# citiususc/veryfasttree

Measured on AMD Instinct MI355X. Metric: profile-ops/sec, higher is better.
Workload: dtype f32; 1 GPU; c4_1M_x200_nt_tophits; n_seqs=1000000, n_pos=200, active_nodes=750000, top_k=2000

## Files before the change

veryfasttree_amd/csrc/vft_api.hip:

```cpp
#include <hip/hip_runtime.h>
#include <csignal>
#include <unistd.h>

#include <cmath>
#include <cstdarg>
#include <cstdio>
#include <cstdlib>
#include <cstring>
#include <new>
#include <algorithm>
#include <utility>
#include <vector>
#include <chrono>

#include "../../include/vft_hip.h"
#include "vft_owned.h"
#include "vft_staging.h"
#define VFT_PAIR_STAGE_CAP 2048
#include "vft_kernels_ml.h"

VFT_ML_HEAVY_INSTANCES(extern)
#include "vft_kernels_ml_long.h"
VFT_ML_LONG_INSTANCES(extern)
#include "vft_kernels_nj.h"
// ... 2015 lines not shown
                return fail(c, VFT_ERR_TIMEOUT, "no selection result after %.0f s (the stream is still busy)", c->waitLimitS);
        }
    }
}

template <typename REAL, typename HIT>
static int run_select(vft_ctx *c, int K, const int64_t *queries, int64_t lo, int64_t hi, int32_t k) {
    std::vector<SelSlot> hs((size_t) K);
    for (int s = 0; s < K; s++) {
        const vft_ctx::SweepSlotHost &h = c->slots[(size_t) s];
        SelSlot &d = hs[(size_t) s];
        d.crit = h.swCrit;
        d.dist = h.swDist;
        d.weight = h.swWeight;
        d.partMin = h.partMin;
        d.partMax = h.partMax;
        d.sel = h.sel;
        d.slices = h.slices;
        d.candKey = h.candKey;
        d.candId = h.candId;
        d.hits = h.dRes + sizeof(SelectHeader);
        d.hdr = (SelectHeader *) h.dRes;
        d.hostHdr = (SelectHeader *) h.hResDev;
        d.hostHits = h.hResDev + sizeof(SelectHeader);
        d.query = queries[s];
        d.nPart = h.nPart;
        d.pad = 0;
    }
    Stage st;
    if (int r = st.open(c, hs.size() * sizeof(SelSlot), Stage::RING_ONLY)) return r;
    st.put(0, hs.data(), hs.size() * sizeof(SelSlot));
    const SelSlot *slots = st.dev<const SelSlot>(0);
    auto round = [&](const SelSlot *sl, unsigned ny, int first, int s0) -> int {
        const unsigned long long seq = ++c->signalSeq;
        launch((k_select_hist<REAL>), dim3(VFT_SEL_WGS, ny), dim3(VFT_WG), 0, c->stream, sl, lo, hi, first);
        launch((k_select_collect<REAL>), dim3(VFT_SEL_WGS, ny), dim3(VFT_WG), 0, c->stream, sl, lo, hi, (unsigned int) k);
        launch((k_select_rank<REAL, HIT>), dim3(VFT_CAND_CAP * VFT_RANK_LANES / VFT_WG, ny), dim3(VFT_WG), 0, c->stream, sl, k, lo, hi, (long long) seq);
        LAUNCHCHK(c);
        return wait_headers(c, s0, (int) ny, seq);
    };
    if (int r = round(slots, (unsigned) K, 1, 0)) return r;
    for (int s = 0; s < K; s++) {
        const SelectHeader *h = (const SelectHeader *) c->slots[(size_t) s].hRes;
        for (int level = 0; h->overflow; level++) {
            if (level == VFT_MAX_LEVEL)
                return fail(c, VFT_ERR_STATE, "top-k select: more than %d hits tied at the k-th criterion", VFT_CAND_CAP);
            launch(k_select_refine, dim3(1, 1), dim3(1), 0, c->stream, slots + s);
            if (int r = round(slots + s, 1u, 0, s)) return r;
        }
    }
    return VFT_OK;
}

#ifdef VFT_SELECT_PHASES
extern "C" int vft_debug_select_phases(vft_ctx *c, unsigned long long *out, int64_t nOut) {
    if (nOut != (int64_t) VFT_SELPH_ROWS * VFT_SELPH_SEEDS * VFT_SELPH_MARKS) return fail(c, VFT_ERR_INVALID, "vft_debug_select_phases: %d x %d x %d words", VFT_SELPH_ROWS, VFT_SELPH_SEEDS, VFT_SELPH_MARKS);
    HIPCHK(c, hipStreamSynchronize(c->stream));
    HIPCHK(c, hipMemcpyFromSymbol(out, HIP_SYMBOL(vft_selph), sizeof(vft_selph)));
    static const unsigned long long zero[VFT_SELPH_ROWS][VFT_SELPH_SEEDS][VFT_SELPH_MARKS] = {};
    HIPCHK(c, hipMemcpyToSymbol(HIP_SYMBOL(vft_selph), zero, sizeof(zero)));
    return VFT_OK;
}
#endif

static int sweep_one(vft_ctx *c, int slot, int64_t query, int64_t nActive, int64_t nDiffAllow, double totdiam, bool staged = false) {
    if (int r = flush_pending(c)) return r;
    const int64_t lo = c->shardLo, hi = c->shardHi < c->maxnode ? c->shardHi : c->maxnode;
    if (c->maxStamp - nActive > nDiffAllow)
        if (int r = launch_out_distances(c, nullptr, 0, nActive, nDiffAllow, totdiam, false)) return r;
    if ((int64_t) c->hNOut[query] - nActive > nDiffAllow) {
        if (nActive > c->maxStamp) c->maxStamp = nActive;
        SweepArgs s{};
        s.nActive = nActive;
        s.nDiffAllow = nDiffAllow;
        s.totdiam = totdiam;
        s.force = 0;
        VFT_DISPATCH(c, launch((k_out_distance_one<REAL, NC>), dim3(1), dim3(VFT_WG), pw_lds_bytes(c) / c->pwWaves, c->stream,
                               arena<REAL>(c), query, s));
        LAUNCHCHK(c);
    }
    SweepArgs s{};
    s.query = query;
    s.lo = lo;
    s.hi = hi;
    s.nActive = nActive;
    s.nDiffAllow = nDiffAllow;
    s.totdiam = totdiam;
    s.queryIsLeaf = query < c->d.nSeqs ? 1 : 0;
#ifdef VFT_ABLATE
    if (const char *dbg = getenv("VFT_SWEEP_ABLATE")) s.pad = atoi(dbg);
#endif
    const int64_t span = hi > lo ? hi - lo : 0;
    const bool ntPath = c->cfg.n_codes == 4 && !c->hasDm;
    const unsigned grid = ntPath ? sweep_nt_grid(c, s, !s.queryIsLeaf) : cdiv(span > 0 ? span : 1, VFT_WG);
    c->slots[(size_t) slot].nPart = (int) grid;
    const int64_t nPosPad = (int64_t) c->d.nChunk * VFT_CHUNK;
    if (c->cfg.n_codes == 4 && !c->hasDm) {
        if (c->cfg.precision == 4) {
            const QueryBuf<float> Q = staged ? qbuf_slot<float>(c, slot) : qbuf<float>(c, 0);
            if (!staged) launch((k_extract_query<float, 4>), dim3(cdiv(nPosPad, 256)), dim3(256), 0, c->stream, arena<float>(c), query, Q);
            if (s.queryIsLeaf) launch_sweep_nt<float, MODE_CRIT_LEAFQ>(c, s, grid, Q, true, slot);
            else launch_sweep_nt<float, MODE_CRIT>(c, s, grid, Q, true, slot);
        } else {
            const QueryBuf<double> Q = staged ? qbuf_slot<double>(c, slot) : qbuf<double>(c, 0);
            if (!staged) launch((k_extract_query<double, 4>), dim3(cdiv(nPosPad, 256)), dim3(256), 0, c->stream, arena<double>(c), query, Q);
            if (s.queryIsLeaf) launch_sweep_nt<double, MODE_CRIT_LEAFQ>(c, s, grid, Q, true, slot);
// ... 8 lines not shown
            const unsigned wgrid = (unsigned) std::min<int64_t>(cdiv(span > 0 ? span : 1, c->pwWaves), 256 * 16);
            c->slots[(size_t) slot].nPart = (int) wgrid;
            VFT_DISPATCH(c, (launch((k_sweep_wave<REAL, NC>), dim3(wgrid), dim3(64 * c->pwWaves), pw_lds_bytes(c), c->stream,
                                    arena<REAL>(c), s, sweepout<REAL>(c, slot))));
        } else {
            VFT_DISPATCH(c, (launch((k_sweep_generic<REAL, NC>), dim3(grid), dim3(VFT_WG), 0, c->stream,
                                    arena<REAL>(c), s, sweepout<REAL>(c, slot))));
        }
        kernel_event(c);
        kernel_event(c);
    }
    LAUNCHCHK(c);
    return VFT_OK;
}

template <typename REAL, int S>
static int sweep_group(vft_ctx *c, bool leafSeeds, const int *slotOf, const int64_t *queries, int64_t nActive, int64_t nDiffAllow, double totdiam, const void *mq, const void *lq) {
    SweepArgs s{};
    s.query = queries[slotOf[0]];
    s.lo = c->shardLo;
    s.hi = c->shardHi < c->maxnode ? c->shardHi : c->maxnode;
    s.nActive = nActive;
    s.nDiffAllow = nDiffAllow;
    s.totdiam = totdiam;
    s.queryIsLeaf = leafSeeds ? 1 : 0;
    const unsigned grid = sweep_nt_grid(c, s, !leafSeeds);
    MultiLeafQ<REAL, S> M;
    for (int q = 0; q < S; q++) {
        M.Q[q] = qbuf_slot<REAL>(c, slotOf[q]);
        M.O[q] = sweepout<REAL>(c, slotOf[q]);
        M.query[q] = queries[slotOf[q]];
        c->slots[(size_t) slotOf[q]].nPart = (int) grid;
    }
    M.mq = (const REAL *) mq;
    M.lq = (const uint32_t *) lq;
    kernel_event(c);
    if (grid && leafSeeds) launch((k_sweep_nt_leafq_multi<REAL, S>), dim3(grid), dim3(VFT_WG), 0, c->stream, arena<REAL>(c), M, s);
    if (grid && !leafSeeds) launch((k_sweep_nt_profq_multi<REAL, S>), dim3(grid), dim3(VFT_WG), 0, c->stream, arena<REAL>(c), M, s);
    kernel_event(c);
    kernel_event(c);
    if (c->timeKernels) c->kevSweeps += S - 1;
    LAUNCHCHK(c);
    return VFT_OK;
}

static bool mixed_sweep_fits(vft_ctx *c) {
    SweepArgs s{};
    s.lo = c->shardLo;
    s.hi = c->shardHi < c->maxnode ? c->shardHi : c->maxnode;
    const unsigned grid = sweep_nt_grid(c, s, true);
    if (!s.nLeafWG || grid == (unsigned) s.nLeafWG || s.hi <= s.leafEnd) return false;
    if (c->rs != 4) return false;
    const int64_t N = slot_nodes(c, 1);
    return (int64_t) cdiv(s.leafEnd - s.lo, VFT_WG) + (int64_t) (grid - (unsigned) s.nLeafWG) <= (int64_t) cdiv(N, VFT_WG);
}

template <typename REAL>
static int sweep_mixed(vft_ctx *c, const int *leafPos, const int *profPos, const int64_t *queries, int64_t nActive, int64_t nDiffAllow, double totdiam, const void *mq, const void *lq) {
    constexpr int S = 4;
    MixedArgs<REAL, S, S> a;
    memset((void *) &a, 0, sizeof(a));
    a.A = arena<REAL>(c);
    SweepArgs &s = a.s;
    s.query = queries[profPos[0]];
    s.lo = c->shardLo;
    s.hi = c->shardHi < c->maxnode ? c->shardHi : c->maxnode;
    s.nActive = nActive;
    s.nDiffAllow = nDiffAllow;
    s.totdiam = totdiam;
    s.queryIsLeaf = 0;
    const unsigned gridP = sweep_nt_grid(c, s, true);
    a.nInt = (int32_t) (gridP - (unsigned) s.nLeafWG);
    a.nLeafHeavy = (int32_t) cdiv(s.leafEnd - s.lo, VFT_WG);
    for (int q = 0; q < S; q++) {
        a.M.L.Q[q] = qbuf_slot<REAL>(c, leafPos[q]);
        a.M.L.O[q] = sweepout<REAL>(c, leafPos[q]);
        a.M.L.query[q] = queries[leafPos[q]];
        c->slots[(size_t) leafPos[q]].nPart = a.nLeafHeavy + a.nInt;
        a.M.P.Q[q] = qbuf_slot<REAL>(c, profPos[q]);
        a.M.P.O[q] = sweepout<REAL>(c, profPos[q]);
        a.M.P.query[q] = queries[profPos[q]];
        c->slots[(size_t) profPos[q]].nPart = (int) gridP;
    }
    a.M.L.mq = nullptr;
    a.M.L.lq = (const uint32_t *) lq;
    a.M.P.mq = (const REAL *) mq;
    a.M.P.lq = nullptr;
    kernel_event(c);
    launch((k_sweep_nt_mixed_multi<REAL, S, S>), dim3((unsigned) (a.nInt + a.nLeafHeavy + s.nLeafWG)), dim3(VFT_WG), 0, c->stream, a);
    kernel_event(c);
    kernel_event(c);
    if (c->timeKernels) c->kevSweeps += 2 * S - 1;
    LAUNCHCHK(c);
    return VFT_OK;
}

static int no_slot(vft_ctx *c) { return fail(c, VFT_ERR_STATE, "the context has no sweep buffers (vft_create failed)"); }

static int sweep_args_ok(vft_ctx *c, int64_t query, int64_t nActive, int32_t k) {
    if (c->slots.empty()) return no_slot(c);
    if (!c->leavesUp) return fail(c, VFT_ERR_STATE, "vft_sweep before vft_upload_leaves");
    if (query < 0 || query >= c->maxnode || nActive < 3 || k < 0 || k > c->hitsCap)
        return fail(c, VFT_ERR_INVALID, "vft_sweep: bad arguments (query %lld, nActive %lld, k %d)", (long long) query,
                    (long long) nActive, (int) k);
    return VFT_OK;
}

extern "C" int vft_sweep(vft_ctx *c, int64_t query, int64_t nActive, int64_t nDiffAllow, double totdiam, int32_t k,
                         void *hits, void *dHitsOut, int64_t *bestJ) {
    if (!c) return VFT_ERR_INVALID;
    if (int r = sweep_args_ok(c, query, nActive, k)) return r;
    if (int r = sweep_one(c, 0, query, nActive, nDiffAllow, totdiam)) return r;
    if (k == 0) return VFT_OK;
    if (bestJ && k < 2) return fail(c, VFT_ERR_INVALID, "vft_sweep: best_j needs k >= 2");
    const int64_t lo = c->shardLo, hi = c->shardHi < c->maxnode ? c->shardHi : c->maxnode;
    int r;
    if (c->cfg.precision == 4) r = run_select<float, vft_hit_f32>(c, 1, &query, lo, hi, k);
    else r = run_select<double, vft_hit_f64>(c, 1, &query, lo, hi, k);
    if (r) return r;
    const size_t hb = (size_t) k * (c->cfg.precision == 4 ? sizeof(vft_hit_f32) : sizeof(vft_hit_f64));
    const vft_ctx::SweepSlotHost &h = c->slots[0];
    if (dHitsOut) HIPCHK(c, hipMemcpyAsync(dHitsOut, h.dRes + sizeof(SelectHeader), hb, hipMemcpyDeviceToDevice, c->stream));
    if (hits) memcpy(hits, h.hRes + sizeof(SelectHeader), hb);
    if (bestJ) *bestJ = (int64_t) ((const SelectHeader *) h.hRes)->bestJ;
    return VFT_OK;
}

struct SeedGroup {
    int pos[4];
    int n;
    bool leaf;
};

extern "C" int vft_sweep_batch(vft_ctx *c, int32_t nSeeds, const int64_t *queries, int64_t nActive, int64_t nDiffAllow,
                               double totdiam, int32_t k, void *hits, void *dHitsOut, int64_t *bestJ) {
    if (!c || !queries || nSeeds < 1 || nSeeds > VFT_MAX_SLOTS || k < 1) return VFT_ERR_INVALID;
    if (bestJ && k < 2) return fail(c, VFT_ERR_INVALID, "vft_sweep_batch: best_j needs k >= 2");
    for (int s = 0; s < nSeeds; s++)
        if (int r = sweep_args_ok(c, queries[s], nActive, k)) return r;
    if (int r = ensure_slots(c, nSeeds)) return r;
    const bool staged = c->cfg.n_codes == 4 && !c->hasDm && nSeeds > 1;
    std::vector<SeedGroup> groups;
// ... 2006 lines not shown
```

veryfasttree_amd/csrc/vft_kernels_nj.h:

```cpp
#pragma once
#include "vft_device.h"

#define VFT_WG 256

template <typename REAL>
struct QueryBuf {
    REAL *w;
    uint8_t *code;
    REAL *f;
    uint4 *enc;
    double2 *tab;
};

template <typename REAL>
__device__ __forceinline__ void vft_query_tab(const QueryBuf<REAL> &q, int64_t p, REAL wq, const REAL *f) {
#pragma unroll
    for (int c = 0; c < 5; c++) {
        double2 v = make_double2(0.0, 0.0);
        if (c < 4 && wq > 0) {
            const double wgt = (double) wq;
            const double piece = 1.0 - (double) f[c < 4 ? c : 0];
            v = make_double2(wgt * piece, wgt);
        }
        q.tab[p * 5 + c] = v;
// ... 113 lines not shown
    int64_t query;
    int64_t lo, hi;
    int64_t nActive, nDiffAllow;
    double totdiam;
    int32_t queryIsLeaf;
    int32_t force;
    int32_t nLeafWG;
    int32_t pad;
    int64_t leafEnd;
    int64_t heavyLo;
};

template <typename REAL>
struct SweepOut {
    REAL *dist, *weight, *crit;
    REAL *partMin, *partMax;
};

template <typename REAL, int NWAVES>
__device__ __forceinline__ void vft_block_minmax_n(REAL cmin, REAL cmax, REAL *partMin, REAL *partMax, int part) {
    __shared__ REAL smin[NWAVES], smax[NWAVES];
#pragma unroll
    for (int off = 32; off > 0; off >>= 1) {
        const REAL a = __shfl_xor(cmin, off, 64), b = __shfl_xor(cmax, off, 64);
        cmin = a < cmin ? a : cmin;
        cmax = b > cmax ? b : cmax;
    }
    if ((threadIdx.x & 63) == 0) {
        smin[threadIdx.x >> 6] = cmin;
        smax[threadIdx.x >> 6] = cmax;
    }
    __syncthreads();
    if (threadIdx.x == 0) {
#pragma unroll
        for (int w = 1; w < NWAVES; w++) {
            cmin = smin[w] < cmin ? smin[w] : cmin;
            cmax = smax[w] > cmax ? smax[w] : cmax;
        }
        partMin[part] = cmin;
        partMax[part] = cmax;
    }
}
template <typename REAL>
__device__ __forceinline__ void vft_block_minmax(REAL cmin, REAL cmax, REAL *partMin, REAL *partMax, int part) {
    vft_block_minmax_n<REAL, VFT_WG / 64>(cmin, cmax, partMin, partMax, part);
}

enum { MODE_CRIT = 0, MODE_OUTDIST = 1, MODE_CRIT_LEAFQ = 2 };

__device__ __forceinline__ void vft_seq_counts(const uint4 a, const uint4 b, int &nUse, int &nSame) {
    const uint32_t x = a.x & b.x, y = a.y & b.y, z = a.z & b.z, w = a.w & b.w;
    nUse += __popc(x & 0x10101010u) + __popc(y & 0x10101010u) + __popc(z & 0x10101010u) + __popc(w & 0x10101010u);
    nSame += __popc(x & 0x0F0F0F0Fu) + __popc(y & 0x0F0F0F0Fu) + __popc(z & 0x0F0F0F0Fu) + __popc(w & 0x0F0F0F0Fu);
}

#ifndef VFT_SUB
#define VFT_SUB 8
#endif
__device__ __forceinline__ uint32_t vft_query_code(const uint8_t *code, int64_t p0, int b) {
    const uint32_t w = vft_uniform_load<uint32_t>((const uint32_t *) (code + p0 + (b & ~3)));
    return (w >> ((b & 3) * 8)) & 0xFFu;
}
template <typename REAL>
__device__ __forceinline__ uint32_t vft_query_code(const QueryBuf<REAL> &Q, int64_t p0, int b) {
    return vft_query_code(Q.code, p0, b);
}

template <typename REAL, bool QLEAF>
struct IntChunk {
    REAL w[VFT_SUB];
    REAL f[VFT_SUB][QLEAF ? 1 : 4];
};

typedef unsigned int __attribute__((ext_vector_type(4))) vft_u4_t;
typedef unsigned int __attribute__((ext_vector_type(2))) vft_u2_t;
typedef const __attribute__((address_space(4))) vft_u4_t *vft_smask_t;
typedef const __attribute__((address_space(4))) vft_u2_t *vft_soff_t;

#ifdef VFT_ABLATE
#define VFT_ABLATE_BITS(s) ((s).pad)
#else
#define VFT_ABLATE_BITS(s) 0
#endif

template <typename REAL, bool QLEAF>
__device__ __forceinline__ void vft_int_chunk_load(IntChunk<REAL, QLEAF> &r, int c, int sub, const uint4 codes,
                                                   const REAL *wT, vft_smask_t mM, vft_soff_t mO, const REAL *fT,
                                                   const QueryBuf<REAL> &Q, int dbg = 0) {
    const int64_t p0 = (int64_t) c * VFT_CHUNK + sub * VFT_SUB;
    vft_u4_t mk[VFT_SUB];
    vft_u2_t of[VFT_SUB];
#pragma unroll
    for (int b = 0; b < VFT_SUB; b++) {
        mk[b] = mM[p0 + b];
        of[b] = mO[p0 + b];
    }
#pragma unroll
    for (int b = 0; b < VFT_SUB; b++) {
        const unsigned long long mv = ((unsigned long long) mk[b].y << 32) | mk[b].x;
        const unsigned long long mw = ((unsigned long long) mk[b].w << 32) | mk[b].z;
        const bool hv = __builtin_amdgcn_inverse_ballot_w64(mv) && !(dbg & 1);
        const bool hw = __builtin_amdgcn_inverse_ballot_w64(mw) && !(dbg & 2);
        const uint32_t slotV = __builtin_amdgcn_mbcnt_hi(mk[b].y, __builtin_amdgcn_mbcnt_lo(mk[b].x, of[b].x));
        const uint32_t slotW = __builtin_amdgcn_mbcnt_hi(mk[b].w, __builtin_amdgcn_mbcnt_lo(mk[b].z, of[b].y));
        const uint32_t cd = vft_byte(codes, sub * VFT_SUB + b);
        r.w[b] = (hv || cd != VFT_NOCODE_) ? (REAL) 1 : (REAL) 0;
// ... 742 lines not shown
    vft_ul4_t rec;
    if constexpr (SL > 0) rec = *(const __attribute__((address_space(4))) vft_ul4_t *) (lq + p0);
    QueryCol<float, SP> cur, nxt;
    vft_query_col_load<float, SP>(cur, mq, p0);
#pragma unroll
    for (int b = 0; b < SUB; b++) {
        if (b + 1 < SUB) vft_query_col_load<float, SP>(nxt, mq, p0 + b + 1);
        __builtin_amdgcn_sched_barrier(0);
        const double P0 = 1.0 - (double) ca.f[b].x, P1 = 1.0 - (double) ca.f[b].y, P2 = 1.0 - (double) ca.f[b].z, P3 = 1.0 - (double) ca.f[b].w;
        {
            double wgt[SP], prod[SP];
#pragma unroll
            for (int q = 0; q < SP; q++) {
                const float ww = cur.w[q] * ca.w[b];
                wgt[q] = (double) ww;
            }
            vft_ipiece_mul<SP>(prod, P0, P1, P2, P3, wgt, cur.codes);
#pragma unroll
            for (int q = 0; q < SP; q++) {
                if (__builtin_expect((cur.codes & (0x40u << (8 * q))) != 0, 0)) {
                    const UVec4<float>::type pr = cur.f[q] * ca.f[b];
                    double head = 1.0 - (double) pr.x;
                    head -= (double) pr.y;
                    head -= (double) pr.z;
                    prod[q] = wgt[q] * (head - (double) pr.w);
                }
                denomP[q] += wgt[q];
                topP[q] += prod[q];
                asm volatile("" : "+v"(topP[q]), "+v"(denomP[q]));
            }
        }
        if constexpr (SL > 0) {
            const unsigned long long w2 = b < 2 ? rec.x : b < 4 ? rec.y : b < 6 ? rec.z : rec.w;
            const uint32_t cw = (uint32_t) (w2 >> (32 * (b & 1)));
            const double wd = (double) ca.w[b];
            const double w4[4] = {wd, wd, wd, wd};
            double prod[SL > 0 ? SL : 1];
            vft_ipiece_mul<SL>(prod, P0, P1, P2, P3, w4, cw);
#pragma unroll
            for (int q = 0; q < SL; q++) {
                if (__builtin_expect((cw & (0x40u << (8 * q))) != 0, 0)) continue;
                denomL[q] += wd;
                topL[q] += prod[q];
                asm volatile("" : "+v"(topL[q]), "+v"(denomL[q]));
            }
        }
        __builtin_amdgcn_sched_barrier(0);
        if (b + 1 < SUB) cur = nxt;
    }
}
#endif

#define VFT_PTILE_M 112
template <int NBT, int S>
__device__ __forceinline__ void vft_leaf_table_chunk_multi(const double2 *row, const uint4 *t, double (*top)[S], double (*denom)[S]) {
    constexpr int GC = NBT * S >= 8 ? 1 : NBT * S >= 4 ? 2 : 4;
#pragma unroll
    for (int g = 0; g < VFT_CHUNK; g += GC) {
        double2 v[NBT][GC][S];
#pragma unroll
        for (int bt = 0; bt < NBT; bt++)
#pragma unroll
            for (int q = 0; q < GC; q++) {
                const int idx = __ffs((int) (vft_byte(t[bt], g + q) | 0x10u)) - 1;
#pragma unroll
                for (int sd = 0; sd < S; sd++) v[bt][q][sd] = row[sd * (VFT_PTILE_M * 5) + (g + q) * 5 + idx];
            }
#pragma unroll
        for (int q = 0; q < GC; q++)
#pragma unroll
            for (int bt = 0; bt < NBT; bt++)
#pragma unroll
                for (int sd = 0; sd < S; sd++) {
                    denom[bt][sd] += v[bt][q][sd].y;
                    top[bt][sd] += v[bt][q][sd].x;
                }
    }
}

template <typename REAL, int NBT, int S>
__device__ __forceinline__ void vft_leaf_table_walk_multi(const Arena<REAL> &A, const MultiLeafQ<REAL, S> &M, double2 *tab, const int64_t *tj,
                                                          double (*top)[S], double (*denom)[S]) {
    const int tid = threadIdx.x;
    const int64_t nPos = A.d.nPos;
    const uint4 *lp[NBT];
#pragma unroll
    for (int bt = 0; bt < NBT; bt++) lp[bt] = A.leafT + vft_leaf_idx(A.d, tj[bt] >> 6, 0, (int) (tj[bt] & 63));
    for (int64_t p0 = 0; p0 < nPos; p0 += VFT_PTILE_M) {
        __syncthreads();
        {
            const int64_t nTab = ((int64_t) A.d.nChunk * VFT_CHUNK - p0) * 5;
#pragma unroll
            for (int sd = 0; sd < S; sd++)
                for (int e = tid; e < VFT_PTILE_M * 5; e += VFT_WG)
                    tab[sd * (VFT_PTILE_M * 5) + e] = e < nTab ? M.Q[sd].tab[p0 * 5 + e] : make_double2(0.0, 0.0);
        }
        __syncthreads();
        const int c0 = (int) (p0 / VFT_CHUNK);
        const int c1 = (int) (((p0 + VFT_PTILE_M < nPos ? p0 + VFT_PTILE_M : nPos) + VFT_CHUNK - 1) / VFT_CHUNK);
        uint4 ta[NBT], tb[NBT];
#pragma unroll
        for (int bt = 0; bt < NBT; bt++) ta[bt] = lp[bt][(int64_t) c0 * VFT_TILE];
        for (int c = c0; c < c1; c += 2) {
            const int cb = c + 1 < c1 ? c + 1 : c, ca = c + 2 < c1 ? c + 2 : c;
#pragma unroll
            for (int bt = 0; bt < NBT; bt++) tb[bt] = lp[bt][(int64_t) cb * VFT_TILE];
            __builtin_amdgcn_sched_barrier(0);
            vft_leaf_table_chunk_multi<NBT, S>(tab + (int64_t) (c - c0) * VFT_CHUNK * 5, ta, top, denom);
#pragma unroll
            for (int bt = 0; bt < NBT; bt++) ta[bt] = lp[bt][(int64_t) ca * VFT_TILE];
            __builtin_amdgcn_sched_barrier(0);
            if (c + 1 < c1) vft_leaf_table_chunk_multi<NBT, S>(tab + (int64_t) (c + 1 - c0) * VFT_CHUNK * 5, tb, top, denom);
        }
    }
}

template <typename REAL, int S>
__device__ __forceinline__ void vft_leaf_table_wg_multi(const Arena<REAL> &A, const MultiLeafQ<REAL, S> &M, const SweepArgs &s, int64_t base,
                                                        REAL *cmin, REAL *cmax) {
    constexpr int NB = VFT_LEAF_SPAN / VFT_WG, NW = VFT_WG / 64, NBT = 2;
    __shared__ double2 tab[S * VFT_PTILE_M * 5];
    __shared__ unsigned short list[VFT_LEAF_SPAN];
    __shared__ int segCnt[NB * NW];
    const int tid = threadIdx.x, wave = tid >> 6;
    unsigned long long bal[NB];
#pragma unroll
    for (int r = 0; r < NB; r++) {
        const int64_t j = base + r * VFT_WG + tid;
        bool active = false;
        if (j < s.leafEnd) {
            active = A.parent[j] < 0;
            if (!active) {
#pragma unroll
                for (int q = 0; q < S; q++) {
                    M.O[q].dist[j] = (REAL) 1e20;
                    M.O[q].crit[j] = (REAL) 1e20;
                    M.O[q].weight[j] = 0;
                }
            }
        }
        bal[r] = __ballot(active);
        if ((tid & 63) == 0) segCnt[r * NW + wave] = __popcll(bal[r]);
    }
    __syncthreads();
    int nAct = 0, off[NB];
#pragma unroll
    for (int seg = 0; seg < NB * NW; seg++) {
#pragma unroll
        for (int r = 0; r < NB; r++)
            if (seg == r * NW + wave) off[r] = nAct;
        nAct += segCnt[seg];
    }
#pragma unroll
    for (int r = 0; r < NB; r++) {
        const int rank = (int) __builtin_amdgcn_mbcnt_hi((unsigned int) (bal[r] >> 32), __builtin_amdgcn_mbcnt_lo((unsigned int) bal[r], 0u));
        if ((bal[r] >> (tid & 63)) & 1ull) list[off[r] + rank] = (unsigned short) (r * VFT_WG + tid);
    }
    __syncthreads();
    for (int r0 = 0; r0 < nAct; r0 += NBT * VFT_WG) {
        int64_t tj[NBT];
        double top[NBT][S], denom[NBT][S];
#pragma unroll
        for (int bt = 0; bt < NBT; bt++) {
            const int idx = r0 + bt * VFT_WG + tid;
            tj[bt] = base + list[idx < nAct ? idx : 0];
// ... 27 lines not shown
}
template <typename REAL>
__device__ __forceinline__ SweepOut<REAL> vft_karg_out(const VFT_KARG SweepOut<REAL> *p) {
    typedef __attribute__((address_space(1))) REAL *gp_t;
    SweepOut<REAL> o;
    o.dist = (REAL *) (gp_t) p->dist;
    o.weight = (REAL *) (gp_t) p->weight;
    o.crit = (REAL *) (gp_t) p->crit;
    o.partMin = (REAL *) (gp_t) p->partMin;
    o.partMax = (REAL *) (gp_t) p->partMax;
    return o;
}
template <typename REAL, int S>
__device__ __forceinline__ void vft_karg_sentinels(const VFT_KARG MultiLeafQ<REAL, S> *M, int64_t j) {
#pragma unroll
    for (int q = 0; q < S; q++) {
        const SweepOut<REAL> O = vft_karg_out<REAL>(&M->O[q]);
        O.dist[j] = (REAL) 1e20;
        O.crit[j] = (REAL) 1e20;
        O.weight[j] = 0;
    }
}
template <typename REAL, int S>
__device__ __forceinline__ void vft_block_minmax_karg(REAL *cmin, REAL *cmax, const VFT_KARG MultiLeafQ<REAL, S> *M, int part,
                                                      REAL (*smin)[VFT_WG / 64], REAL (*smax)[VFT_WG / 64]) {
    constexpr int NW = VFT_WG / 64;
#pragma unroll
    for (int q = 0; q < S; q++) {
#pragma unroll
        for (int off = 32; off > 0; off >>= 1) {
            const REAL a = __shfl_xor(cmin[q], off, 64), b = __shfl_xor(cmax[q], off, 64);
            cmin[q] = a < cmin[q] ? a : cmin[q];
            cmax[q] = b > cmax[q] ? b : cmax[q];
        }
        if ((threadIdx.x & 63) == 0) {
            smin[q][threadIdx.x >> 6] = cmin[q];
            smax[q][threadIdx.x >> 6] = cmax[q];
        }
    }
    __syncthreads();
    if (threadIdx.x < S) {
        const int q = threadIdx.x;
        REAL lo = smin[q][0], hi = smax[q][0];
#pragma unroll
        for (int w = 1; w < NW; w++) {
            lo = smin[q][w] < lo ? smin[q][w] : lo;
            hi = smax[q][w] > hi ? smax[q][w] : hi;
        }
        const SweepOut<REAL> O = vft_karg_out<REAL>(&M->O[q]);
        O.partMin[part] = lo;
        O.partMax[part] = hi;
    }
}

template <typename REAL, int S>
__global__ __launch_bounds__(VFT_WG, sizeof(REAL) == 4 ? 3 : 2) void k_sweep_nt_profq_multi(Arena<REAL> A, MultiLeafQ<REAL, S> M, SweepArgs s) {
    constexpr int SUB = 8;
    __shared__ REAL smin[S][VFT_WG / 64], smax[S][VFT_WG / 64];
    const int nT = s.nLeafWG, nHeavy = (int) gridDim.x - nT, blk = (int) blockIdx.x;
    REAL cmin[S], cmax[S];
#pragma unroll
    for (int q = 0; q < S; q++) {
        cmin[q] = (REAL) 1e30;
        cmax[q] = (REAL) -1e30;
    }
    if (blk >= nHeavy) {
        const int span = blk - nHeavy;
        vft_leaf_table_wg_multi<REAL, S>(A, M, s, s.lo + (int64_t) span * VFT_LEAF_SPAN, cmin, cmax);
        vft_block_minmax_multi<REAL, S>(cmin, cmax, M.O, span);
        return;
    }
    const int wg = nHeavy - 1 - blk;
    const int64_t j = s.heavyLo + (int64_t) wg * VFT_WG + threadIdx.x;
    const int lane = (int) (j & 63);
    const int64_t tile = j >> 6;
    constexpr size_t offM = (sizeof(Arena<REAL>) + alignof(MultiLeafQ<REAL, S>) - 1) / alignof(MultiLeafQ<REAL, S>) * alignof(MultiLeafQ<REAL, S>);
    const VFT_KARG MultiLeafQ<REAL, S> *M0 = vft_kernarg<MultiLeafQ<REAL, S>>(offM);
    bool work = false;
    if (j < s.hi && !(nT && j < s.leafEnd)) {
        work = A.parent[j] < 0;
        if (!work) vft_karg_sentinels<REAL, S>(M0, j);
    }
    double top[S], denom[S];
#pragma unroll
    for (int q = 0; q < S; q++) top[q] = denom[q] = 0;
    const VFT_KARG MultiLeafQ<REAL, S> *M1 = vft_kernarg<MultiLeafQ<REAL, S>>(offM);
    if (work) {
        const REAL *mq = M1->mq;
        vft_for_column_groups<REAL, SUB>(A, tile, lane, [&](const IntChunkAll<REAL, SUB> &ca, int64_t p0) {
#if VFT_SHARED_PIECES
            if constexpr (sizeof(REAL) == 4 && S == 4) vft_int_chunk_consume_shared<0, S, SUB>(ca, p0, mq, nullptr, top, denom, nullptr, nullptr);
            else
#endif
                vft_int_chunk_consume_prof<REAL, S, SUB, sizeof(REAL) == 4>(ca, p0, mq, top, denom);
            vft_pin_sums<S>(top, denom);
        });
    }
    const VFT_KARG MultiLeafQ<REAL, S> *Mk = vft_kernarg<MultiLeafQ<REAL, S>>(offM);
    if (work) {
#pragma unroll
        for (int q = 0; q < S; q++) {
            const REAL weight = (REAL) (denom[q] > 0 ? denom[q] : 0.01);
            const REAL dist = (REAL) (denom[q] > 0 ? top[q] / denom[q] : 1.0);
            SweepArgs sq = s;
            sq.query = Mk->query[q];
            vft_sweep_finish<REAL, MODE_CRIT>(A, sq, vft_karg_out<REAL>(&Mk->O[q]), j, dist, weight, false, cmin[q], cmax[q]);
        }
    }
    vft_block_minmax_karg<REAL, S>(cmin, cmax, vft_kernarg<MultiLeafQ<REAL, S>>(offM), nT + wg, smin, smax);
}

template <typename REAL, int SL, int SP>
struct MixedQ {
    MultiLeafQ<REAL, SL> L;
    MultiLeafQ<REAL, SP> P;
};
template <typename REAL, int SL, int SP>
struct MixedArgs {
    Arena<REAL> A;
    SweepArgs s;
    int32_t nInt, nLeafHeavy;
    MixedQ<REAL, SL, SP> M;
};
template <typename REAL, int SL, int SP>
__global__ __launch_bounds__(VFT_WG, sizeof(REAL) == 4 ? 3 : 2) void k_sweep_nt_mixed_multi(MixedArgs<REAL, SL, SP> a) {
    typedef MixedArgs<REAL, SL, SP> Args;
    constexpr int SUB = 8, NW = VFT_WG / 64;
    constexpr size_t offL = offsetof(Args, M) + offsetof(decltype(Args::M), L), offP = offsetof(Args, M) + offsetof(decltype(Args::M), P);
    __shared__ REAL smin[SL + SP][NW], smax[SL + SP][NW];
    const Arena<REAL> &A = a.A;
    const SweepArgs &s = a.s;
    const int blk = (int) blockIdx.x, nInt = a.nInt, nLH = a.nLeafHeavy, nT = s.nLeafWG;
    REAL cminP[SP], cmaxP[SP], cminL[SL], cmaxL[SL];
#pragma unroll
    for (int q = 0; q < SP; q++) {
        cminP[q] = (REAL) 1e30;
        cmaxP[q] = (REAL) -1e30;
    }
#pragma unroll
    for (int q = 0; q < SL; q++) {
        cminL[q] = (REAL) 1e30;
        cmaxL[q] = (REAL) -1e30;
    }
    if (blk >= nInt + nLH) {
        const int span = blk - nInt - nLH;
        const VFT_KARG MultiLeafQ<REAL, SP> *Pk = vft_kernarg<MultiLeafQ<REAL, SP>>(offP);
        MultiLeafQ<REAL, SP> M;
#pragma unroll
        for (int q = 0; q < SP; q++) {
            M.Q[q].w = Pk->Q[q].w;
            M.Q[q].code = Pk->Q[q].code;
            M.Q[q].f = Pk->Q[q].f;
            M.Q[q].enc = Pk->Q[q].enc;
            M.Q[q].tab = Pk->Q[q].tab;
            M.O[q] = vft_karg_out<REAL>(&Pk->O[q]);
            M.query[q] = Pk->query[q];
        }
        M.mq = Pk->mq;
        vft_leaf_table_wg_multi<REAL, SP>(A, M, s, s.lo + (int64_t) span * VFT_LEAF_SPAN, cminP, cmaxP);
        vft_block_minmax_karg<REAL, SP>(cminP, cmaxP, vft_kernarg<MultiLeafQ<REAL, SP>>(offP), span, smin, smax);
        return;
    }
    if (blk >= nInt) {
        const int wg = nLH - 1 - (blk - nInt);
        const int64_t j = s.lo + (int64_t) wg * VFT_WG + threadIdx.x;
        const VFT_KARG MultiLeafQ<REAL, SL> *Lk = vft_kernarg<MultiLeafQ<REAL, SL>>(offL);
        bool work = false;
        if (j < s.leafEnd) {
            work = A.parent[j] < 0;
            if (!work) vft_karg_sentinels<REAL, SL>(Lk, j);
        }
        if (work) {
            const uint4 *enc[SL];
            int nUse[SL], nSame[SL];
#pragma unroll
            for (int q = 0; q < SL; q++) {
                enc[q] = Lk->Q[q].enc;
                nUse[q] = nSame[q] = 0;
            }
            const int lane = (int) (j & 63);
            const int64_t tile = j >> 6;
            for (int c = 0; c < A.d.nChunk; c++) {
                const uint4 t = A.leafT[vft_leaf_idx(A.d, tile, c, lane)];
#pragma unroll
                for (int q = 0; q < SL; q++) vft_seq_counts(t, enc[q][c], nUse[q], nSame[q]);
            }
#pragma unroll
            for (int q = 0; q < SL; q++) {
                const double top = (double) (nUse[q] - nSame[q]);
                const REAL weight = (REAL) (double) nUse[q];
                const REAL dist = (REAL) (nUse[q] > 0 ? top / (double) nUse[q] : 1.0);
                SweepArgs sq = s;
                sq.query = Lk->query[q];
                vft_sweep_finish<REAL, MODE_CRIT>(A, sq, vft_karg_out<REAL>(&Lk->O[q]), j, dist, weight, true, cminL[q], cmaxL[q]);
            }
        }
        vft_block_minmax_karg<REAL, SL>(cminL, cmaxL, vft_kernarg<MultiLeafQ<REAL, SL>>(offL), wg, smin, smax);
        return;
    }
    const int wg = nInt - 1 - blk;
    const int64_t j = s.heavyLo + (int64_t) wg * VFT_WG + threadIdx.x;
    const int lane = (int) (j & 63);
    const int64_t tile = j >> 6;
    const VFT_KARG MixedQ<REAL, SL, SP> *M0 = vft_kernarg<MixedQ<REAL, SL, SP>>(offsetof(Args, M));
    bool work = false;
    if (j < s.hi && j >= s.leafEnd) {
        work = A.parent[j] < 0;
        if (!work) {
            vft_karg_sentinels<REAL, SP>(&M0->P, j);
            vft_karg_sentinels<REAL, SL>(&M0->L, j);
        }
    }
    double topP[SP], denomP[SP], topL[SL], denomL[SL];
#pragma unroll
    for (int q = 0; q < SP; q++) topP[q] = denomP[q] = 0;
#pragma unroll
    for (int q = 0; q < SL; q++) topL[q] = denomL[q] = 0;
    const VFT_KARG MixedQ<REAL, SL, SP> *M1 = vft_kernarg<MixedQ<REAL, SL, SP>>(offsetof(Args, M));
    if (work) {
        const REAL *mq = M1->P.mq;
        LeafCodes<SL> lc;
#if VFT_SEED_CODE_RECORDS
        lc.lq = M1->L.lq;
#else
#pragma unroll
        for (int q = 0; q < SL; q++) lc.code[q] = M1->L.Q[q].code;
#endif
        vft_for_column_groups<REAL, SUB>(A, tile, lane, [&](const IntChunkAll<REAL, SUB> &ca, int64_t p0) {
#if VFT_SHARED_PIECES
            if constexpr (sizeof(REAL) == 4) {
                vft_int_chunk_consume_shared<SL, SP, SUB>(ca, p0, mq, lc.lq, topP, denomP, topL, denomL);
                vft_pin_sums<SP>(topP, denomP);
                vft_pin_sums<SL>(topL, denomL);
                __builtin_amdgcn_sched_barrier(0);
                return;
            }
#endif
            vft_int_chunk_consume_prof<REAL, SP, SUB, sizeof(REAL) == 4>(ca, p0, mq, topP, denomP);
            vft_pin_sums<SP>(topP, denomP);
            __builtin_amdgcn_sched_barrier(0);
            vft_int_chunk_consume_all<REAL, SL, SUB, true, sizeof(REAL) == 4>(ca, p0, lc, topL, denomL);
            vft_pin_sums<SL>(topL, denomL);
            __builtin_amdgcn_sched_barrier(0);
        });
    }
    const VFT_KARG MixedQ<REAL, SL, SP> *Mk = vft_kernarg<MixedQ<REAL, SL, SP>>(offsetof(Args, M));
    if (work) {
#pragma unroll
        for (int q = 0; q < SP; q++) {
            const REAL weight = (REAL) (denomP[q] > 0 ? denomP[q] : 0.01);
            const REAL dist = (REAL) (denomP[q] > 0 ? topP[q] / denomP[q] : 1.0);
            SweepArgs sq = s;
            sq.query = Mk->P.query[q];
            vft_sweep_finish<REAL, MODE_CRIT>(A, sq, vft_karg_out<REAL>(&Mk->P.O[q]), j, dist, weight, false, cminP[q], cmaxP[q]);
        }
#pragma unroll
        for (int q = 0; q < SL; q++) {
            const REAL weight = (REAL) (denomL[q] > 0 ? denomL[q] : 0.01);
            const REAL dist = (REAL) (denomL[q] > 0 ? topL[q] / denomL[q] : 1.0);
            SweepArgs sq = s;
            sq.query = Mk->L.query[q];
            vft_sweep_finish<REAL, MODE_CRIT>(A, sq, vft_karg_out<REAL>(&Mk->L.O[q]), j, dist, weight, false, cminL[q], cmaxL[q]);
        }
    }
    vft_block_minmax_karg<REAL, SP>(cminP, cmaxP, vft_kernarg<MultiLeafQ<REAL, SP>>(offP), nT + wg, smin, smax);
    vft_block_minmax_karg<REAL, SL>(cminL, cmaxL, vft_kernarg<MultiLeafQ<REAL, SL>>(offL), nLH + wg, smin + SP, smax + SP);
}

template <typename REAL, int NC>
__device__ __forceinline__ void vft_pair_generic(const Arena<REAL> &A, int64_t i, int64_t j, bool jIsOut, REAL &dist,
                                                 REAL &weight) {
    const int64_t nPos = A.d.nPos;
    if (!jIsOut && i < A.d.nSeqs && j < A.d.nSeqs) {
        double top = 0;
        int64_t nUse = 0;
        int nDiff = 0;
        const int li = (int) (i & 63), lj = (int) (j & 63);
        for (int c = 0; c < A.d.nChunk; c++) {
            const uint4 a = A.leafT[vft_leaf_idx(A.d, i >> 6, c, li)];
            const uint4 b = A.leafT[vft_leaf_idx(A.d, j >> 6, c, lj)];
            for (int t = 0; t < VFT_CHUNK; t++) {
                if ((int64_t) c * VFT_CHUNK + t >= nPos) break;
                const int ca = vft_decode<NC>(vft_byte(a, t)), cb = vft_decode<NC>(vft_byte(b, t));
                if (ca != VFT_NOCODE_ && cb != VFT_NOCODE_) {
                    nUse++;
                    if (A.dmDist) top += (double) A.dmDist[ca * NC + cb];
                    else if (ca != cb) nDiff++;
                }
            }
        }
        if (!A.dmDist) top = (double) nDiff;
        weight = (REAL) (double) nUse;
        dist = (REAL) (nUse > 0 ? top / (double) nUse : 1.0);
        return;
    }
    double top = 0, denom = 0;
    for (int64_t p = 0; p < nPos; p++) {
        Col<REAL, NC> c1, c2;
        vft_load_col<REAL, NC>(A, i, p, c1);
        if (jIsOut) {
            c2.w = A.outW[p];
            c2.code = VFT_NOCODE_;
            c2.vec = c2.w > 0;
#pragma unroll
            for (int k = 0; k < NC; k++) c2.f[k] = A.outF[p * NC + k];
        } else {
            vft_load_col<REAL, NC>(A, j, p, c2);
        }
        if (c1.w > 0 && c2.w > 0) {
            const REAL ww = c1.w * c2.w;
            const double wgt = (double) ww;
            denom += wgt;
            const double piece = vft_piece<REAL, NC>(A, c1, c2, (jIsOut && A.outCD) ? A.outCD + p * NC : nullptr);
            top += wgt * piece;
        }
    }
    weight = (REAL) (denom > 0 ? denom : 0.01);
    dist = (REAL) (denom > 0 ? top / denom : 1.0);
}
// ... 1257 lines not shown
```

Baseline: 16.01 billion profile-ops/s.

## Share leaf compaction and encoding walk between leaf and profile queries in mixed sweep

In the mixed sweep kernel, the leaf-query work over leaf rows now happens inside the profile-query leaf-table workgroups. The active-leaf compaction and the leaf tile loads are done once and reused for both query types, with the leaf-query match counts packed into one 32-bit word. This removes the separate leaf-heavy workgroups and their duplicate reads of leaf encodings, and shrinks the grid. The cost is more register pressure and longer per-workgroup work in the shared walk, and a new nPos < 65536 limit, since nUse and nSame are packed into 16 bits each. An optional, off-by-default per-workgroup clock probe is added as well.

```diff
diff --git a/veryfasttree_amd/csrc/vft_api.hip b/veryfasttree_amd/csrc/vft_api.hip
--- a/veryfasttree_amd/csrc/vft_api.hip
+++ b/veryfasttree_amd/csrc/vft_api.hip
@@ -2091,6 +2091,18 @@
     return VFT_OK;
 }
 
+#ifdef VFT_SWEEP_WG_CLOCKS
+extern "C" int vft_debug_sweep_wg_clocks(vft_ctx *c, unsigned long long *out, int64_t nOut) {
+    if (nOut != (int64_t) VFT_SWCLK_MAX * 3) return fail(c, VFT_ERR_INVALID, "vft_debug_sweep_wg_clocks: %d x 3 words", VFT_SWCLK_MAX);
+    HIPCHK(c, hipStreamSynchronize(c->stream));
+    HIPCHK(c, hipMemcpyFromSymbol(out, HIP_SYMBOL(vft_swclk), sizeof(vft_swclk)));
+    void *dev = nullptr;
+    HIPCHK(c, hipGetSymbolAddress(&dev, HIP_SYMBOL(vft_swclk)));
+    HIPCHK(c, hipMemset(dev, 0, sizeof(vft_swclk)));
+    return VFT_OK;
+}
+#endif
+
 #ifdef VFT_SELECT_PHASES
 extern "C" int vft_debug_select_phases(vft_ctx *c, unsigned long long *out, int64_t nOut) {
     if (nOut != (int64_t) VFT_SELPH_ROWS * VFT_SELPH_SEEDS * VFT_SELPH_MARKS) return fail(c, VFT_ERR_INVALID, "vft_debug_select_phases: %d x %d x %d words", VFT_SELPH_ROWS, VFT_SELPH_SEEDS, VFT_SELPH_MARKS);
@@ -2205,7 +2217,11 @@
     if (!s.nLeafWG || grid == (unsigned) s.nLeafWG || s.hi <= s.leafEnd) return false;
     if (c->rs != 4) return false;
     const int64_t N = slot_nodes(c, 1);
+#if VFT_SHARED_LEAF_WALK
+    return c->d.nPos < 65536 && (int64_t) grid <= (int64_t) cdiv(N, VFT_WG);
+#else
     return (int64_t) cdiv(s.leafEnd - s.lo, VFT_WG) + (int64_t) (grid - (unsigned) s.nLeafWG) <= (int64_t) cdiv(N, VFT_WG);
+#endif
 }
 
 template <typename REAL>
@@ -2224,12 +2240,17 @@
     s.queryIsLeaf = 0;
     const unsigned gridP = sweep_nt_grid(c, s, true);
     a.nInt = (int32_t) (gridP - (unsigned) s.nLeafWG);
+#if VFT_SHARED_LEAF_WALK
+    const int nPartL = (int) gridP, nLeafWGs = s.nLeafWG;
+#else
     a.nLeafHeavy = (int32_t) cdiv(s.leafEnd - s.lo, VFT_WG);
+    const int nPartL = a.nLeafHeavy + a.nInt, nLeafWGs = a.nLeafHeavy + s.nLeafWG;
+#endif
     for (int q = 0; q < S; q++) {
         a.M.L.Q[q] = qbuf_slot<REAL>(c, leafPos[q]);
         a.M.L.O[q] = sweepout<REAL>(c, leafPos[q]);
         a.M.L.query[q] = queries[leafPos[q]];
-        c->slots[(size_t) leafPos[q]].nPart = a.nLeafHeavy + a.nInt;
+        c->slots[(size_t) leafPos[q]].nPart = nPartL;
         a.M.P.Q[q] = qbuf_slot<REAL>(c, profPos[q]);
         a.M.P.O[q] = sweepout<REAL>(c, profPos[q]);
         a.M.P.query[q] = queries[profPos[q]];
@@ -2240,7 +2261,7 @@
     a.M.P.mq = (const REAL *) mq;
     a.M.P.lq = nullptr;
     kernel_event(c);
-    launch((k_sweep_nt_mixed_multi<REAL, S, S>), dim3((unsigned) (a.nInt + a.nLeafHeavy + s.nLeafWG)), dim3(VFT_WG), 0, c->stream, a);
+    launch((k_sweep_nt_mixed_multi<REAL, S, S>), dim3((unsigned) (a.nInt + nLeafWGs)), dim3(VFT_WG), 0, c->stream, a);
     kernel_event(c);
     kernel_event(c);
     if (c->timeKernels) c->kevSweeps += 2 * S - 1;
diff --git a/veryfasttree_amd/csrc/vft_kernels_nj.h b/veryfasttree_amd/csrc/vft_kernels_nj.h
--- a/veryfasttree_amd/csrc/vft_kernels_nj.h
+++ b/veryfasttree_amd/csrc/vft_kernels_nj.h
@@ -189,6 +189,13 @@
     const uint32_t x = a.x & b.x, y = a.y & b.y, z = a.z & b.z, w = a.w & b.w;
     nUse += __popc(x & 0x10101010u) + __popc(y & 0x10101010u) + __popc(z & 0x10101010u) + __popc(w & 0x10101010u);
     nSame += __popc(x & 0x0F0F0F0Fu) + __popc(y & 0x0F0F0F0Fu) + __popc(z & 0x0F0F0F0Fu) + __popc(w & 0x0F0F0F0Fu);
+}
+
+__device__ __forceinline__ void vft_seq_counts_packed(const uint4 a, const uint4 b, uint32_t &cnt) {
+    const uint32_t x = a.x & b.x, y = a.y & b.y, z = a.z & b.z, w = a.w & b.w;
+    const uint32_t same = __popc(x & 0x0F0F0F0Fu) + __popc(y & 0x0F0F0F0Fu) + __popc(z & 0x0F0F0F0Fu) + __popc(w & 0x0F0F0F0Fu);
+    cnt += __popc(x & 0x10101010u) + __popc(y & 0x10101010u) + __popc(z & 0x10101010u) + __popc(w & 0x10101010u);
+    cnt += same << 16;
 }
 
 #ifndef VFT_SUB
@@ -1037,9 +1044,9 @@
 #endif
 
 #define VFT_PTILE_M 112
-template <int NBT, int S>
+template <int NBT, int S, int GCF = 0>
 __device__ __forceinline__ void vft_leaf_table_chunk_multi(const double2 *row, const uint4 *t, double (*top)[S], double (*denom)[S]) {
-    constexpr int GC = NBT * S >= 8 ? 1 : NBT * S >= 4 ? 2 : 4;
+    constexpr int GC = GCF ? GCF : NBT * S >= 8 ? 1 : NBT * S >= 4 ? 2 : 4;
 #pragma unroll
     for (int g = 0; g < VFT_CHUNK; g += GC) {
         double2 v[NBT][GC][S];
@@ -1063,9 +1070,40 @@
     }
 }
 
-template <typename REAL, int NBT, int S>
+template <int SL>
+struct LeafEncChunk {
+    uint4 e[SL > 0 ? SL : 1];
+};
+template <int SL>
+__device__ __forceinline__ void vft_leaf_enc_load(LeafEncChunk<SL> &d, const uint4 *const *enc, int c) {
+    typedef uint32_t __attribute__((ext_vector_type(4))) u4_t;
+    typedef const __attribute__((address_space(4))) u4_t *cp_t;
+#pragma unroll
+    for (int q = 0; q < SL; q++) {
+        const u4_t v = *((cp_t) enc[q] + c);
+        d.e[q] = make_uint4(v.x, v.y, v.z, v.w);
+    }
+}
+template <int NBT, int S, int SL>
+__device__ __forceinline__ void vft_leaf_walk_chunk(const double2 *row, const uint4 *t, double (*top)[S], double (*denom)[S],
+                                                    const LeafEncChunk<SL> &e, uint32_t (*cnt)[SL > 0 ? SL : 1]) {
+    if constexpr (SL > 0) {
+#pragma unroll
+        for (int bt = 0; bt < NBT; bt++) vft_leaf_table_chunk_multi<1, S, 1>(row, t + bt, top + bt, denom + bt);
+        __builtin_amdgcn_sched_barrier(0);
+#pragma unroll
+        for (int bt = 0; bt < NBT; bt++)
+#pragma unroll
+            for (int q = 0; q < SL; q++) vft_seq_counts_packed(t[bt], e.e[q], cnt[bt][q]);
+    } else {
+        vft_leaf_table_chunk_multi<NBT, S>(row, t, top, denom);
+    }
+}
+
+template <typename REAL, int NBT, int S, int SL = 0>
 __device__ __forceinline__ void vft_leaf_table_walk_multi(const Arena<REAL> &A, const MultiLeafQ<REAL, S> &M, double2 *tab, const int64_t *tj,
-                                                          double (*top)[S], double (*denom)[S]) {
+                                                          double (*top)[S], double (*denom)[S], const uint4 *const *enc = nullptr,
+                                                          uint32_t (*cnt)[SL > 0 ? SL : 1] = nullptr) {
     const int tid = threadIdx.x;
     const int64_t nPos = A.d.nPos;
     const uint4 *lp[NBT];
@@ -1084,18 +1122,22 @@
         const int c0 = (int) (p0 / VFT_CHUNK);
         const int c1 = (int) (((p0 + VFT_PTILE_M < nPos ? p0 + VFT_PTILE_M : nPos) + VFT_CHUNK - 1) / VFT_CHUNK);
         uint4 ta[NBT], tb[NBT];
+        LeafEncChunk<SL> ea, eb;
 #pragma unroll
         for (int bt = 0; bt < NBT; bt++) ta[bt] = lp[bt][(int64_t) c0 * VFT_TILE];
+        if constexpr (SL > 0) vft_leaf_enc_load<SL>(ea, enc, c0);
         for (int c = c0; c < c1; c += 2) {
             const int cb = c + 1 < c1 ? c + 1 : c, ca = c + 2 < c1 ? c + 2 : c;
 #pragma unroll
             for (int bt = 0; bt < NBT; bt++) tb[bt] = lp[bt][(int64_t) cb * VFT_TILE];
+            if constexpr (SL > 0) vft_leaf_enc_load<SL>(eb, enc, cb);
             __builtin_amdgcn_sched_barrier(0);
-            vft_leaf_table_chunk_multi<NBT, S>(tab + (int64_t) (c - c0) * VFT_CHUNK * 5, ta, top, denom);
+            vft_leaf_walk_chunk<NBT, S, SL>(tab + (int64_t) (c - c0) * VFT_CHUNK * 5, ta, top, denom, ea, cnt);
 #pragma unroll
             for (int bt = 0; bt < NBT; bt++) ta[bt] = lp[bt][(int64_t) ca * VFT_TILE];
+            if constexpr (SL > 0) vft_leaf_enc_load<SL>(ea, enc, ca);
             __builtin_amdgcn_sched_barrier(0);
-            if (c + 1 < c1) vft_leaf_table_chunk_multi<NBT, S>(tab + (int64_t) (c + 1 - c0) * VFT_CHUNK * 5, tb, top, denom);
+            if (c + 1 < c1) vft_leaf_walk_chunk<NBT, S, SL>(tab + (int64_t) (c + 1 - c0) * VFT_CHUNK * 5, tb, top, denom, eb, cnt);
         }
     }
 }
@@ -1229,6 +1271,107 @@
         O.partMax[part] = hi;
     }
 }
+
+#ifdef VFT_NO_SHARED_LEAF_WALK
+#define VFT_SHARED_LEAF_WALK 0
+#else
+#define VFT_SHARED_LEAF_WALK 1
+#endif
+#if VFT_SHARED_LEAF_WALK
+template <typename REAL, int SL, int SP>
+__device__ __forceinline__ void vft_leaf_table_wg_mixed(const Arena<REAL> &A, const MultiLeafQ<REAL, SP> &P, size_t offL, const SweepArgs &s,
+                                                        int64_t base, REAL *cminP, REAL *cmaxP, REAL *cminL, REAL *cmaxL) {
+    constexpr int NB = VFT_LEAF_SPAN / VFT_WG, NW = VFT_WG / 64, NBT = 2;
+    __shared__ double2 tab[SP * VFT_PTILE_M * 5];
+    __shared__ unsigned short list[VFT_LEAF_SPAN];
+    __shared__ int segCnt[NB * NW];
+    const int tid = threadIdx.x, wave = tid >> 6;
+    const VFT_KARG MultiLeafQ<REAL, SL> *L0 = vft_kernarg<MultiLeafQ<REAL, SL>>(offL);
+    unsigned long long bal[NB];
+#pragma unroll
+    for (int r = 0; r < NB; r++) {
+        const int64_t j = base + r * VFT_WG + tid;
+        bool active = false;
+        if (j < s.leafEnd) {
+            active = A.parent[j] < 0;
+            if (!active) {
+#pragma unroll
+                for (int q = 0; q < SP; q++) {
+                    P.O[q].dist[j] = (REAL) 1e20;
+                    P.O[q].crit[j] = (REAL) 1e20;
+                    P.O[q].weight[j] = 0;
+                }
+                vft_karg_sentinels<REAL, SL>(L0, j);
+            }
+        }
+        bal[r] = __ballot(active);
+        if ((tid & 63) == 0) segCnt[r * NW + wave] = __popcll(bal[r]);
+    }
+    __syncthreads();
+    int nAct = 0, off[NB];
+#pragma unroll
+    for (int seg = 0; seg < NB * NW; seg++) {
+#pragma unroll
+        for (int r = 0; r < NB; r++)
+            if (seg == r * NW + wave) off[r] = nAct;
+        nAct += segCnt[seg];
+    }
+#pragma unroll
+    for (int r = 0; r < NB; r++) {
+        const int rank = (int) __builtin_amdgcn_mbcnt_hi((unsigned int) (bal[r] >> 32), __builtin_amdgcn_mbcnt_lo((unsigned int) bal[r], 0u));
+        if ((bal[r] >> (tid & 63)) & 1ull) list[off[r] + rank] = (unsigned short) (r * VFT_WG + tid);
+    }
+    __syncthreads();
+    for (int r0 = 0; r0 < nAct; r0 += NBT * VFT_WG) {
+        int64_t tj[NBT];
+        double top[NBT][SP], denom[NBT][SP];
+        uint32_t cnt[NBT][SL];
+#pragma unroll
+        for (int bt = 0; bt < NBT; bt++) {
+            const int idx = r0 + bt * VFT_WG + tid;
+            tj[bt] = base + list[idx < nAct ? idx : 0];
+#pragma unroll
+            for (int q = 0; q < SP; q++) top[bt][q] = denom[bt][q] = 0;
+#pragma unroll
+            for (int q = 0; q < SL; q++) cnt[bt][q] = 0;
+        }
+        {
+            const VFT_KARG MultiLeafQ<REAL, SL> *L1 = vft_kernarg<MultiLeafQ<REAL, SL>>(offL);
+            const uint4 *enc[SL];
+#pragma unroll
+            for (int q = 0; q < SL; q++) enc[q] = L1->Q[q].enc;
+            if (nAct - r0 <= VFT_WG) vft_leaf_table_walk_multi<REAL, 1, SP, SL>(A, P, tab, tj, top, denom, enc, cnt);
+            else vft_leaf_table_walk_multi<REAL, NBT, SP, SL>(A, P, tab, tj, top, denom, enc, cnt);
+        }
+        const VFT_KARG MultiLeafQ<REAL, SL> *Lk = vft_kernarg<MultiLeafQ<REAL, SL>>(offL);
+#pragma unroll
+        for (int bt = 0; bt < NBT; bt++) {
+            const int idx = r0 + bt * VFT_WG + tid;
+            tj[bt] = base + list[idx < nAct ? idx : 0];
+            if (idx < nAct) {
+#pragma unroll
+                for (int q = 0; q < SP; q++) {
+                    const REAL weight = (REAL) (denom[bt][q] > 0 ? denom[bt][q] : 0.01);
+                    const REAL dist = (REAL) (denom[bt][q] > 0 ? top[bt][q] / denom[bt][q] : 1.0);
+                    SweepArgs sq = s;
+                    sq.query = P.query[q];
+                    vft_sweep_finish<REAL, MODE_CRIT>(A, sq, P.O[q], tj[bt], dist, weight, false, cminP[q], cmaxP[q]);
+                }
+#pragma unroll
+                for (int q = 0; q < SL; q++) {
+                    const int nUse = (int) (cnt[bt][q] & 0xFFFFu), nSame = (int) (cnt[bt][q] >> 16);
+                    const double topq = (double) (nUse - nSame);
+                    const REAL weight = (REAL) (double) nUse;
+                    const REAL dist = (REAL) (nUse > 0 ? topq / (double) nUse : 1.0);
+                    SweepArgs sq = s;
+                    sq.query = Lk->query[q];
+                    vft_sweep_finish<REAL, MODE_CRIT>(A, sq, vft_karg_out<REAL>(&Lk->O[q]), tj[bt], dist, weight, true, cminL[q], cmaxL[q]);
+                }
+            }
+        }
+    }
+}
+#endif
 
 template <typename REAL, int S>
 __global__ __launch_bounds__(VFT_WG, sizeof(REAL) == 4 ? 3 : 2) void k_sweep_nt_profq_multi(Arena<REAL> A, MultiLeafQ<REAL, S> M, SweepArgs s) {
@@ -1296,9 +1439,30 @@
 struct MixedArgs {
     Arena<REAL> A;
     SweepArgs s;
+#if VFT_SHARED_LEAF_WALK
+    int32_t nInt, pad;
+#else
     int32_t nInt, nLeafHeavy;
+#endif
     MixedQ<REAL, SL, SP> M;
 };
+#ifdef VFT_SWEEP_WG_CLOCKS
+#define VFT_SWCLK_MAX 8192
+__device__ unsigned long long vft_swclk[VFT_SWCLK_MAX][3];
+#define VFT_SWCLK_BEGIN() const unsigned long long vft_swclk_t0 = wall_clock64()
+#define VFT_SWCLK_END(kind, worked)                                                                                    \
+    do {                                                                                                               \
+        const int vft_swclk_any = __syncthreads_or((int) (worked));                                                    \
+        if (threadIdx.x == 0 && blockIdx.x < VFT_SWCLK_MAX) {                                                          \
+            vft_swclk[blockIdx.x][0] = (unsigned long long) ((kind) | (vft_swclk_any ? 16 : 0));                       \
+            vft_swclk[blockIdx.x][1] = vft_swclk_t0;                                                                   \
+            vft_swclk[blockIdx.x][2] = wall_clock64();                                                                 \
+        }                                                                                                              \
+    } while (0)
+#else
+#define VFT_SWCLK_BEGIN() ((void) 0)
+#define VFT_SWCLK_END(kind, worked) ((void) 0)
+#endif
 template <typename REAL, int SL, int SP>
 __global__ __launch_bounds__(VFT_WG, sizeof(REAL) == 4 ? 3 : 2) void k_sweep_nt_mixed_multi(MixedArgs<REAL, SL, SP> a) {
     typedef MixedArgs<REAL, SL, SP> Args;
@@ -1307,7 +1471,12 @@
     __shared__ REAL smin[SL + SP][NW], smax[SL + SP][NW];
     const Arena<REAL> &A = a.A;
     const SweepArgs &s = a.s;
+#if VFT_SHARED_LEAF_WALK
+    const int blk = (int) blockIdx.x, nInt = a.nInt, nT = s.nLeafWG;
+#else
     const int blk = (int) blockIdx.x, nInt = a.nInt, nLH = a.nLeafHeavy, nT = s.nLeafWG;
+#endif
+    VFT_SWCLK_BEGIN();
     REAL cminP[SP], cmaxP[SP], cminL[SL], cmaxL[SL];
 #pragma unroll
     for (int q = 0; q < SP; q++) {
@@ -1319,8 +1488,13 @@
         cminL[q] = (REAL) 1e30;
         cmaxL[q] = (REAL) -1e30;
     }
+#if VFT_SHARED_LEAF_WALK
+    if (blk >= nInt) {
+        const int span = nT - 1 - (blk - nInt);
+#else
     if (blk >= nInt + nLH) {
         const int span = blk - nInt - nLH;
+#endif
         const VFT_KARG MultiLeafQ<REAL, SP> *Pk = vft_kernarg<MultiLeafQ<REAL, SP>>(offP);
         MultiLeafQ<REAL, SP> M;
 #pragma unroll
@@ -1334,8 +1508,17 @@
             M.query[q] = Pk->query[q];
         }
         M.mq = Pk->mq;
+#if VFT_SHARED_LEAF_WALK
+        vft_leaf_table_wg_mixed<REAL, SL, SP>(A, M, offL, s, s.lo + (int64_t) span * VFT_LEAF_SPAN, cminP, cmaxP, cminL, cmaxL);
+        vft_block_minmax_karg<REAL, SP>(cminP, cmaxP, vft_kernarg<MultiLeafQ<REAL, SP>>(offP), span, smin, smax);
+        vft_block_minmax_karg<REAL, SL>(cminL, cmaxL, vft_kernarg<MultiLeafQ<REAL, SL>>(offL), span, smin + SP, smax + SP);
+        VFT_SWCLK_END(4, cminP[0] < (REAL) 1e30);
+        return;
+    }
+#else
         vft_leaf_table_wg_multi<REAL, SP>(A, M, s, s.lo + (int64_t) span * VFT_LEAF_SPAN, cminP, cmaxP);
         vft_block_minmax_karg<REAL, SP>(cminP, cmaxP, vft_kernarg<MultiLeafQ<REAL, SP>>(offP), span, smin, smax);
+        VFT_SWCLK_END(3, cminP[0] < (REAL) 1e30);
         return;
     }
     if (blk >= nInt) {
@@ -1373,8 +1556,10 @@
             }
         }
         vft_block_minmax_karg<REAL, SL>(cminL, cmaxL, vft_kernarg<MultiLeafQ<REAL, SL>>(offL), wg, smin, smax);
+        VFT_SWCLK_END(2, cminL[0] < (REAL) 1e30);
         return;
     }
+#endif
     const int wg = nInt - 1 - blk;
     const int64_t j = s.heavyLo + (int64_t) wg * VFT_WG + threadIdx.x;
     const int lane = (int) (j & 63);
@@ -1441,7 +1626,12 @@
         }
     }
     vft_block_minmax_karg<REAL, SP>(cminP, cmaxP, vft_kernarg<MultiLeafQ<REAL, SP>>(offP), nT + wg, smin, smax);
+#if VFT_SHARED_LEAF_WALK
+    vft_block_minmax_karg<REAL, SL>(cminL, cmaxL, vft_kernarg<MultiLeafQ<REAL, SL>>(offL), nT + wg, smin + SP, smax + SP);
+#else
     vft_block_minmax_karg<REAL, SL>(cminL, cmaxL, vft_kernarg<MultiLeafQ<REAL, SL>>(offL), nLH + wg, smin + SP, smax + SP);
+#endif
+    VFT_SWCLK_END(1, cminP[0] < (REAL) 1e30);
 }
 
 template <typename REAL, int NC>
```

New measurement: 17.49 billion profile-ops/s (median of 6 runs). 9.3% higher.
